# Kitsunetic/ERP_match_eightpoint_test

Hardware: AMD Instinct MI355X
Metric: ERP image-pairs/sec (4k x 4k kpts, 10k RANSAC iters); match-set bit-exact (higher is better)
Workload: dtype f32+f64; 1 GPU; configs[1] shape: 4096x4096 kpts/pair, 10000 initial_guess iters, batch of 768 independent pairs per step per GPU; kpts=4096, iters=10000, streams=6, matcher=mfma, parallelism=pair-sharded x1, sampler=glibc replay (seed 1)

## Files before the change

erp_match_eightpoint_test_amd/csrc/kernels.hip:

```cpp
#include <hip/hip_runtime.h>
#include <atomic>

#include <math.h>

#include <algorithm>
#include <type_traits>
#include <utility>
#include <stdint.h>
#include <stdlib.h>

#include "erp_device.hpp"
#include "erp_kernels.hpp"
#include "erp_launch.hpp"

namespace erp {

namespace {

constexpr float kInf = __builtin_huge_valf();

typedef float f32x2 __attribute__((ext_vector_type(2)));
typedef __attribute__((address_space(3))) uint32_t lds_u32;

__constant__ uint32_t c_red[30][31];
// ... 641 lines not shown

template <bool I24, int RS = 8>
__device__ __forceinline__ void split_hits_block(uint32_t (&ring)[31], uint32_t* bm, int lane,
                                                 int i0, int s, const uint64_t (&c)[31]) {
    const uint32_t bm_lane = (uint32_t)(size_t)(lds_u32*)bm + 4u * (uint32_t)lane;
    uint32_t jj[31];
    lat_positions<I24, true>(ring, i0, c, jj);
#pragma unroll
    for (int u = 0; u < 31; u++) {
        const uint32_t j = min(jj[u], (uint32_t)s);
        asm volatile("ds_or_b32 %0, %1" : : "v"(lds_word_addr<RS>(bm_lane, j)), "v"(1u << (j & 31))
                     : "memory");
    }
}

__device__ __forceinline__ void ring_skip_block(uint32_t (&ring)[31]) {
#pragma unroll
    for (int u = 0; u < 31; u++) {
        const int slot = 30 - u;
        ring[slot] = ring[slot] - ring[(slot + 28) % 31];
    }
}

template <typename F>
__device__ __forceinline__ void lat_blocks(int M, int s, int b0, int b1,
                                           const double* __restrict__ rtab, F&& fn) {
    uint64_t ca[31] = {}, cb[31] = {};
    auto live = [&](int b) { return b < b1 && M - 1 - 31 * b >= 1; };
    auto kind = [&](int b) { return live(b) ? lat_kind(M - 1 - 31 * b, s) : 4; };
    int b = b0;
    int ka = kind(b);
    if (live(b) && ka < 4) lat_fetch(rtab, M - 1 - 31 * b, ka, ca);
    while (live(b)) {
        const int kb = kind(b + 1);
        lat_ready(ca);
        if (live(b + 1) && kb < 4) lat_fetch(rtab, M - 1 - 31 * (b + 1), kb, cb);
        fn(b, ka, ca);
        b++;
        if (!live(b)) break;
        ka = kind(b + 1);
        lat_ready(cb);
        if (live(b + 1) && ka < 4) lat_fetch(rtab, M - 1 - 31 * (b + 1), ka, ca);
        fn(b, kb, cb);
        b++;
    }
}

__global__ __launch_bounds__(64 * (kSplitG + 1)) void sampler_split_kernel(
    const int32_t* __restrict__ counts, const uint32_t* __restrict__ wins, int nwaves, int nbw,
    double sample_frac, const double* __restrict__ rtab, uint32_t* __restrict__ selw,
    int32_t* __restrict__ flags, int nalloc) {
    extern __shared__ uint32_t sm[];
    __shared__ int esum[64];
    const int p = blockIdx.y, w = blockIdx.x, lane = threadIdx.x & 63, wv = threadIdx.x >> 6;
    const int M = counts[p];
    const int s = (int)(M * sample_frac);
    if (s < 1 || M < 2) return;
    asm volatile("s_setreg_imm32_b32 hwreg(HW_REG_MODE, 2, 2), 3\n\ts_nop 3" ::: "memory");
#if ERP_SPLIT_STAMPS
    uint64_t ts[8];
    ts[0] = __builtin_amdgcn_s_memtime();
#endif
    const size_t reg = (size_t)nalloc * 64;
    uint32_t* H = sm + (size_t)wv * reg;
    uint32_t* Bm = sm + (size_t)(kSplitG + wv) * reg;
    auto avail = [&](int k) -> uint32_t {
        return k < (s >> 5) ? ~0u : k == (s >> 5) ? (1u << (s & 31)) - 1u : 0u;
    };
    if (wv < kSplitG)
        for (int k = 0; k < nalloc; k++) H[k * 64 + lane] = 0u;
    if (wv == 0) esum[lane] = 0;
    const int nbd = M - 31 - s >= 0 ? (M - 31 - s) / 31 + 1 : 0;
    const int bb = wv < kSplitG ? nbd * wv / kSplitG : nbd;
    const int be = wv < kSplitG ? nbd * (wv + 1) / kSplitG : 0x7fffffff;
    uint32_t ring[31];
    {
        const uint32_t* wi = wins + ((size_t)p * nwaves + w) * 31 * 64 + lane;
#pragma unroll
        for (int t = 0; t < 31; t++) ring[t] = wi[t * 64];
    }
    for (int b = 0; b < bb; b++) ring_skip_block(ring);
#if ERP_SPLIT_STAMPS
    ts[1] = __builtin_amdgcn_s_memtime();
#endif
    __syncthreads();
    uint32_t ring0[31];
#pragma unroll
    for (int t = 0; t < 31; t++) ring0[t] = ring[t];
    if (wv < kSplitG)
        lat_blocks(M, s, bb, be, rtab, [&](int b, int kind, const uint64_t(&c)[31]) {
            const int i0 = M - 1 - 31 * b;
            if (kind == 0) split_hits_block<true>(ring, H, lane, i0, s, c);
            else split_hits_block<false>(ring, H, lane, i0, s, c);
        });
    asm volatile("s_waitcnt lgkmcnt(0)" ::: "memory");
#if ERP_SPLIT_STAMPS
    ts[2] = __builtin_amdgcn_s_memtime();
#endif
    __syncthreads();
#if ERP_SPLIT_STAMPS
    ts[3] = __builtin_amdgcn_s_memtime();
#endif
    const int lim = wv < kSplitG ? wv : kSplitG;
    for (int k0 = 0; k0 < nalloc; k0 += 8) {
        uint32_t e[8] = {0u, 0u, 0u, 0u, 0u, 0u, 0u, 0u};
#pragma unroll
        for (int x = 0; x < kSplitG; x++) {
            if (x < lim) {
#pragma unroll
                for (int q = 0; q < 8; q++)
                    if (k0 + q < nalloc) e[q] |= sm[(size_t)x * reg + (k0 + q) * 64 + lane];
            }
        }
#pragma unroll
        for (int q = 0; q < 8; q++)
            if (k0 + q < nalloc) Bm[(k0 + q) * 64 + lane] = avail(k0 + q) & ~e[q];
    }
#if ERP_SPLIT_STAMPS
    ts[4] = __builtin_amdgcn_s_memtime();
#endif
#pragma unroll
    for (int t = 0; t < 31; t++) ring[t] = ring0[t];
    uint32_t* out = selw + ((size_t)p * nwaves + w) * (size_t)nbw * 64 + lane;
    const int b0 = (M - 1) / 31, u0 = (M - 1) % 31;
    int emitted = 0;
    uint32_t lastw = 0;
    lat_blocks(M, s, bb, be, rtab, [&](int b, int kind, const uint64_t(&c)[31]) {
        const uint32_t word = replay_block_lat<true, 8>(ring, Bm, lane, M - 1 - 31 * b, s, kind, rtab, c);
        emitted += __builtin_popcount(word);
        if (b == b0) lastw = word;
        else out[(size_t)b * 64] = word;
    });
#if ERP_SPLIT_STAMPS
    ts[5] = __builtin_amdgcn_s_memtime();
#endif
    if (wv == kSplitG) {
        if (Bm[lane] & 1u) {
            lastw |= 1u << u0;
            emitted++;
        }
        out[(size_t)b0 * 64] = lastw;
    }
    atomicAdd(&esum[lane], emitted);
    __syncthreads();
    if (wv == kSplitG && esum[lane] != s) atomicOr(&flags[p], 2);
#if ERP_SPLIT_STAMPS
    if (blockIdx.x == 0 && blockIdx.y == 0 && lane == 0)
        printf("split wave %d: skip %d pass1 %d barrier %d init %d pass2 %d (blocks %d..%d, M %d s %d)\n",
               wv, (int)(ts[1] - ts[0]), (int)(ts[2] - ts[1]), (int)(ts[3] - ts[2]),
               (int)(ts[4] - ts[3]), (int)(ts[5] - ts[4]), bb, be, M, s);
#endif
}

__device__ __forceinline__ void philox4x32_10(uint32_t c[4], uint32_t k0, uint32_t k1) {
#pragma unroll
    for (int r = 0; r < 10; r++) {
        const uint64_t p0 = (uint64_t)0xD2511F53u * c[0], p1 = (uint64_t)0xCD9E8D57u * c[2];
        const uint32_t hi0 = (uint32_t)(p0 >> 32), lo0 = (uint32_t)p0;
        const uint32_t hi1 = (uint32_t)(p1 >> 32), lo1 = (uint32_t)p1;
        uint32_t n0, n2;
        asm("v_bitop3_b32 %0, %1, %2, %3 bitop3:0x96" : "=v"(n0) : "v"(hi1), "v"(c[1]), "s"(k0));
        asm("v_bitop3_b32 %0, %1, %2, %3 bitop3:0x96" : "=v"(n2) : "v"(hi0), "v"(c[3]), "s"(k1));
        c[0] = n0;
        c[1] = lo1;
        c[2] = n2;
        c[3] = lo0;
        k0 += 0x9E3779B9u;
        k1 += 0xBB67AE85u;
    }
}

__global__ __launch_bounds__(64) void philox_sampler_kernel(
    const int32_t* __restrict__ counts, int iters, int nwaves, int nbw, double sample_frac,
    uint32_t seed, uint64_t offset, int nwords, uint32_t* __restrict__ selw,
    int32_t* __restrict__ flags) {
    extern __shared__ uint32_t bm[];
    const int p = blockIdx.y, w = blockIdx.x, lane = wave_lane();
    const int M = counts[p];
    const int s = (int)(M * sample_frac);
    if (s < 1 || M < 2) return;
    uint32_t* out = selw + ((size_t)p * nwaves + w) * (size_t)nbw * 64 + lane;
    const int nb = (M - 1) / 31 + 1;
    if ((M + 31) / 32 > nwords) {
        if (lane == 0) atomicOr(&flags[p], 8);
        for (int b = 0; b < nb; b++) out[(size_t)b * 64] = 0u;
        return;
    }
    const int mw = (M + 31) / 32;
    for (int k = 0; k < mw; k++) bm[k * 64 + lane] = 0u;
    const uint64_t h = offset + (uint64_t)(w * 64 + lane);
    uint32_t u[4];
    for (int k0 = 0; k0 < s; k0 += 4) {
        u[0] = (uint32_t)h;
        u[1] = (uint32_t)(h >> 32);
        u[2] = (uint32_t)(k0 >> 2);
        u[3] = 0u;
        philox4x32_10(u, seed, 0x243F6A88u);
#pragma unroll
        for (int q = 0; q < 4; q++) {
            const int k = k0 + q;
            if (k < s) {
                const uint32_t j = (uint32_t)(M - s + k);
                const uint32_t t = __umulhi(u[q], j + 1u);
                const uint32_t old = atomicOr(&bm[(t >> 5) * 64 + lane], 1u << (t & 31));
                if (old & (1u << (t & 31))) atomicOr(&bm[(j >> 5) * 64 + lane], 1u << (j & 31));
            }
        }
    }
    int emitted = 0;
    for (int b = 0; b < nb; b++) {
        const int hi = M - 1 - 31 * b, lo = hi - 30;
        const int l0 = lo < 0 ? 0 : lo;
        const uint32_t a = bm[(l0 >> 5) * 64 + lane];
        const uint32_t c = ((l0 >> 5) + 1) < mw ? bm[((l0 >> 5) + 1) * 64 + lane] : 0u;
        uint32_t win = __builtin_amdgcn_alignbit(c, a, (uint32_t)(l0 & 31));
        if (lo < 0) win = (win << (-lo));
        win &= 0x7fffffffu;
        const uint32_t word = __builtin_bitreverse32(win) >> 1;
        emitted += __builtin_popcount(word);
        out[(size_t)b * 64] = word;
    }
    if (emitted != s) atomicOr(&flags[p], 2);
}

__device__ __forceinline__ void estimate_store(const double* e, double valid_abs,
                                               erp_hypothesis* __restrict__ o,
                                               bool with_e = true) {
    Hyp hy;
    estimate_from_e(e, valid_abs, hy);
#pragma unroll
    for (int k = 0; k < 3; k++) {
        o->R1[k] = hy.R1[k];
        o->R2[k] = hy.R2[k];
        o->T[k] = hy.T[k];
    }
    o->R1_valid = hy.R1_valid;
    o->R2_valid = hy.R2_valid;
    o->inliers = 0;
    if (!with_e) return;
#pragma unroll
    for (int k = 0; k < 9; k++) o->E[k] = hy.E[k];
}

constexpr int kGramLimbs = 6;
constexpr int kGramTiles = 7;
constexpr int kGramN = kGramTiles * 32;
constexpr double kGramScale = 0x1p44;

typedef int i32x4 __attribute__((ext_vector_type(4)));
typedef int i32x16 __attribute__((ext_vector_type(16)));

__device__ __forceinline__ double gram_join(int a0, int a1, int a2, int a3, int a4, int a5) {
    const double lo = __builtin_fma((double)a2, 0x1p-28,
                                    __builtin_fma((double)a1, 0x1p-36, (double)a0 * 0x1p-44));
    const double hi = __builtin_fma((double)a5, 0x1p16, __builtin_fma((double)a4, 0x1p8, (double)a3));
    return __builtin_fma(hi, 0x1p-20, lo);
}

__device__ __forceinline__ int gram_col(int limb, int c) {
    return c < 32 ? limb * 32 + c : 192 + limb * 4 + (c - 32);
}

__device__ __forceinline__ int gram_swz(int n, int u) {
    return n * 32 + ((((u >> 4) ^ (n >> 3)) & 1) << 4) + (u & 15);
}

__global__ __launch_bounds__(256) void gram_limbs_kernel(const int32_t* __restrict__ counts,
                                                         const double* __restrict__ pts,
                                                         int max_nq, int nbw,
                                                         int8_t* __restrict__ limbs) {
    __shared__ __align__(16) int8_t tile[kGramN * 32];
    const int p = blockIdx.y, b = blockIdx.x, tid = threadIdx.x;
    const int M = counts[p];
    if (M < 2 || b > (M - 1) / 31) return;
    for (int k = tid; k < kGramN * 32 / 16; k += 256)
        reinterpret_cast<uint4*>(tile)[k] = make_uint4(0u, 0u, 0u, 0u);
    __syncthreads();
    const double* P = pts + (size_t)p * (max_nq + 1) * 6;
    for (int item = tid; item < 31 * 36; item += 256) {
        const int u = item / 36, c = item - 36 * (item / 36);
        const int i = M - 1 - 31 * b - u;
        if (i < 0) continue;
        const double* pr = P + (size_t)i * 6;
        const int a = c / 6, e = c - 6 * (c / 6);
        const int ai = a < 3 ? 0 : (a < 5 ? 1 : 2), aj = a < 3 ? a : (a < 5 ? a - 2 : 2);
        const int ei = e < 3 ? 0 : (e < 5 ? 1 : 2), ej = e < 3 ? e : (e < 5 ? e - 2 : 2);
        const double LL = pr[ai] * pr[aj], RR = pr[3 + ei] * pr[3 + ej];
        long long q = __double2ll_rn((LL * RR) * kGramScale);
#pragma unroll
        for (int k = 0; k < kGramLimbs; k++) {
            const int d = (int)(int8_t)(q & 0xff);
            tile[gram_swz(gram_col(k, c), u)] = (int8_t)d;
            q = (q - d) >> 8;
        }
    }
    __syncthreads();
    uint4* o = reinterpret_cast<uint4*>(limbs + ((size_t)p * nbw + b) * kGramN * 32);
    for (int k = tid; k < kGramN * 32 / 16; k += 256) o[k] = reinterpret_cast<const uint4*>(tile)[k];
}

#ifndef ERP_GRAM_WAVES
#define ERP_GRAM_WAVES 4
#endif
#ifndef ERP_GRAM_SCHED
#define ERP_GRAM_SCHED 0
#endif
constexpr int kGramWaves = ERP_GRAM_WAVES;
constexpr int kGramWords = 2;
constexpr int kGramWordBytes = kGramN * 32;
constexpr int kGramSelOff = kGramWords * kGramWordBytes;
#ifndef ERP_GRAM_RING
#define ERP_GRAM_RING 3
#endif
#ifndef ERP_GRAM_MINBLOCKS
#define ERP_GRAM_MINBLOCKS 3
#endif
constexpr int kGramPieces = kGramSelOff / 1024;
static_assert(kGramPieces == 14, "14 limb pieces of 1 KB per step");
template <int WT>
struct GramCfg {
    static constexpr int kIters = 32 * kGramWaves * WT;
    static constexpr int kChunks = kIters / 64;
    static constexpr int kSelPW = kGramWords * kChunks / kGramWaves;
    static constexpr int kRing = WT == 1 ? ERP_GRAM_RING : 5;
    static constexpr int kSlotBytes = kGramSelOff + kGramWords * kIters * 4;
    static constexpr int kMinBlocks = WT == 1 ? ERP_GRAM_MINBLOCKS : 2;
    static_assert(kRing >= 3, "ring");
    static_assert(kIters % 64 == 0 && kGramWords * kChunks % kGramWaves == 0 && kGramWaves <= 14,
                  "whole selection-word DMAs per wave");
};
constexpr int gram_pieces_of(int w) {
    return kGramPieces / kGramWaves + (w < kGramPieces % kGramWaves ? 1 : 0);
}
constexpr int gram_piece0(int w) {
    return w * (kGramPieces / kGramWaves) + (w < kGramPieces % kGramWaves ? w : kGramPieces % kGramWaves);
}

typedef __attribute__((address_space(3))) void* lds_vptr;
typedef const __attribute__((address_space(1))) void* glb_vptr;

template <int WT>
__global__ __launch_bounds__(64 * kGramWaves, GramCfg<WT>::kMinBlocks) void gram_mfma_kernel(
    const int32_t* __restrict__ counts, const int8_t* __restrict__ limbs,
    const uint32_t* __restrict__ selw, int iters, int nwaves, int nbw, double sample_frac,
    double* __restrict__ gram, int nhb, double* __restrict__ evec,
    erp_hypothesis* __restrict__ hyps, double valid_abs) {
    using C = GramCfg<WT>;
    __shared__ __align__(16) int8_t lds[C::kRing * C::kSlotBytes];
    const int NB = gridDim.x;
    const int lbk = (NB & 7) ? (int)blockIdx.x : (int)((blockIdx.x & 7) * (NB >> 3) + (blockIdx.x >> 3));
    const int p = lbk / nhb, tid = threadIdx.x, lane = tid & 63, wv = tid >> 6;
    const int M = counts[p];
    const int s = (int)(M * sample_frac);
    if (s < 1 || M < 2) return;
    const int hb = (lbk % nhb) * C::kIters;
    if (hb >= iters) return;
    const int nb = (M - 1) / 31 + 1;
    const int nsteps = (nb + kGramWords - 1) / kGramWords;
    const int h0 = hb + wv * 32 * WT;
    const int r = lane & 31, hh = lane >> 5;
    const int8_t* lg = limbs + (size_t)p * nbw * kGramWordBytes + lane * 16;
    const int lp0 = [&] {
        int v = 0;
#pragma unroll
        for (int w = 0; w < kGramWaves; w++) v = (w == wv) ? gram_piece0(w) : v;
        return v;
    }();
    const bool extra = wv < kGramPieces % kGramWaves;
    const uint32_t* sg[C::kSelPW];
#pragma unroll
    for (int e = 0; e < C::kSelPW; e++) {
        const int d = wv * C::kSelPW + e;
        const int chunk = min((hb >> 6) + d % C::kChunks, nwaves - 1);
        sg[e] = selw + ((size_t)p * nwaves + chunk) * (size_t)nbw * 64 + lane +
                (size_t)(d / C::kChunks) * 64;
    }
    const int soff = kGramSelOff + wv * C::kSelPW * 256;
    auto issue = [&](int step) {
        const int sx = min(step, nsteps - 1);
        int8_t* slot = lds + (step % C::kRing) * C::kSlotBytes;
        const int8_t* src = lg + (size_t)sx * kGramSelOff;
#pragma unroll
        for (int k = 0; k < kGramPieces / kGramWaves; k++)
            __builtin_amdgcn_global_load_lds((glb_vptr)(src + (lp0 + k) * 1024),
                                             (lds_vptr)(slot + (lp0 + k) * 1024), 16, 0, 0);
        if (extra)
            __builtin_amdgcn_global_load_lds(
                (glb_vptr)(src + (lp0 + kGramPieces / kGramWaves) * 1024),
                (lds_vptr)(slot + (lp0 + kGramPieces / kGramWaves) * 1024), 16, 0, 0);
#pragma unroll
        for (int e = 0; e < C::kSelPW; e++)
            __builtin_amdgcn_global_load_lds((glb_vptr)(sg[e] + (size_t)(sx * kGramWords) * 64),
                                             (lds_vptr)(slot + soff + e * 256), 4, 0, 0);
    };
    i32x16 acc[WT][kGramTiles];
#pragma unroll
    for (int w = 0; w < WT; w++)
#pragma unroll
        for (int t = 0; t < kGramTiles; t++)
#pragma unroll
            for (int k = 0; k < 16; k++) acc[w][t][k] = 0;
#pragma unroll
    for (int k = 0; k < C::kRing - 1; k++) issue(k);
    const int boff = r * 32 + (((hh ^ (r >> 3)) & 1) << 4);
    for (int st = 0; st < nsteps; st++) {
        constexpr int kBase = kGramPieces / kGramWaves + C::kSelPW;
        static_assert((kBase + 1) * (C::kRing - 2) <= 63, "vmcnt range");
        if (extra) asm volatile("s_waitcnt vmcnt(%0)" ::"n"((kBase + 1) * (C::kRing - 2)) : "memory");
        else asm volatile("s_waitcnt vmcnt(%0)" ::"n"(kBase * (C::kRing - 2)) : "memory");
        __builtin_amdgcn_s_barrier();
        issue(st + C::kRing - 1);
        const int8_t* slot = lds + (st % C::kRing) * C::kSlotBytes;
        i32x4 bf[kGramWords][kGramTiles];
#pragma unroll
        for (int i = 0; i < kGramWords; i++)
#pragma unroll
            for (int t = 0; t < kGramTiles; t++)
                bf[i][t] = *reinterpret_cast<const i32x4*>(slot + i * kGramWordBytes +
                                                           t * 32 * 32 + boff);
        uint32_t wsel[WT][kGramWords];
#pragma unroll
        for (int w = 0; w < WT; w++)
#pragma unroll
            for (int i = 0; i < kGramWords; i++)
                wsel[w][i] = reinterpret_cast<const uint32_t*>(slot + kGramSelOff)[
                    i * C::kIters + (wv * WT + w) * 32 + r];
        i32x4 a[WT][kGramWords];
#pragma unroll
        for (int w = 0; w < WT; w++)
#pragma unroll
            for (int i = 0; i < kGramWords; i++) {
                const uint32_t wm = (st * kGramWords + i < nb) ? 0xffffu : 0u;
                const uint32_t bits = (wsel[w][i] >> (16 * hh)) & wm;
#pragma unroll
                for (int v = 0; v < 4; v++)
                    a[w][i][v] = (int)((((bits >> (4 * v)) & 0xfu) * 0x00204081u) & 0x01010101u);
            }
#if ERP_GRAM_SCHED
        __builtin_amdgcn_sched_group_barrier(0x100, kGramWords * (kGramTiles + 1), 0);
        __builtin_amdgcn_sched_group_barrier(0x002, 4 * kGramWords * 4, 0);
        __builtin_amdgcn_sched_group_barrier(0x008, kGramWords * kGramTiles, 0);
#endif
#pragma unroll
        for (int i = 0; i < kGramWords; i++)
#pragma unroll
            for (int t = 0; t < kGramTiles; t++)
#pragma unroll
                for (int w = 0; w < WT; w++)
                    acc[w][t] = __builtin_amdgcn_mfma_i32_32x32x32_i8(a[w][i], bf[i][t], acc[w][t], 0, 0, 0);
    }
    asm volatile("s_waitcnt vmcnt(0)" ::: "memory");
    double* go = gram + (size_t)p * 36 * iters;
    if (evec && s >= 9) {
        constexpr int kStg = C::kIters + 1;
        static_assert(36 * kStg * 8 <= C::kRing * C::kSlotBytes, "Gram stage fits the ring");
        double* stg = reinterpret_cast<double*>(lds);
        __syncthreads();
#pragma unroll
        for (int w = 0; w < WT; w++)
#pragma unroll
        for (int k = 0; k < 16; k++) {
            const int row = (wv * WT + w) * 32 + (k & 3) + 8 * (k >> 2) + 4 * hh;
            static_assert(kGramLimbs == 6, "gram_join takes six limbs");
            const int x = acc[w][kGramLimbs][k];
            int y[kGramLimbs];
#pragma unroll
            for (int t = 0; t < kGramLimbs; t++) y[t] = __shfl(x, (lane & 32) + 4 * t + (r & 3), 64);
            stg[r * kStg + row] = gram_join(acc[w][0][k], acc[w][1][k], acc[w][2][k], acc[w][3][k],
                                            acc[w][4][k], acc[w][5][k]);
            if (r < 4) stg[(32 + r) * kStg + row] = gram_join(y[0], y[1], y[2], y[3], y[4], y[5]);
        }
        __syncthreads();
        if (wv >= C::kIters / 64) return;
        const int hl = wv * 64 + lane, h = hb + hl;
        double e[9];
        const bool ok = gram_min_eigvec9_inv(stg, kStg, hl, e);
        if (h >= iters) return;
        if (!ok) {
            e[0] = __builtin_nan("");
#pragma unroll 4
            for (int k = 0; k < 36; k++) go[(size_t)k * iters + h] = stg[k * kStg + hl];
        } else if (hyps) {
            estimate_store(e, valid_abs, hyps + (size_t)p * iters + h);
            evec[(size_t)p * 9 * iters + h] = 0.0;
            return;
        }
        double* eo = evec + (size_t)p * 9 * iters + h;
#pragma unroll
        for (int k = 0; k < 9; k++) eo[(size_t)k * iters] = e[k];
        return;
    }
#pragma unroll
    for (int w = 0; w < WT; w++)
#pragma unroll
    for (int k = 0; k < 16; k++) {
        const int row = w * 32 + (k & 3) + 8 * (k >> 2) + 4 * hh;
        const int x = acc[w][kGramLimbs][k];
        int y[kGramLimbs];
#pragma unroll
        for (int t = 0; t < kGramLimbs; t++) y[t] = __shfl(x, (lane & 32) + 4 * t + (r & 3), 64);
        if (h0 + row < iters) {
            go[(size_t)r * iters + h0 + row] = gram_join(acc[w][0][k], acc[w][1][k], acc[w][2][k],
                                                         acc[w][3][k], acc[w][4][k], acc[w][5][k]);
            if (r < 4)
                go[(size_t)(32 + r) * iters + h0 + row] = gram_join(y[0], y[1], y[2], y[3], y[4], y[5]);
        }
    }
}

__global__ __launch_bounds__(64) void samples_kernel(const int32_t* __restrict__ counts,
                                                     const uint32_t* __restrict__ selw, int iters,
                                                     int nwaves, int nbw, int idx_stride,
                                                     double sample_frac,
                                                     int32_t* __restrict__ samples) {
    const int p = blockIdx.y, lane = wave_lane();
    const int h = blockIdx.x * 64 + lane;
    const int M = counts[p];
    const int s = (int)(M * sample_frac);
    if (s < 1 || M < 2 || h >= iters) return;
    const uint32_t* sp = selw + ((size_t)p * nwaves + blockIdx.x) * (size_t)nbw * 64 + lane;
    int32_t* o = samples + ((size_t)p * iters + h) * idx_stride;
    int n = 0;
    for (int b = 0; b <= (M - 1) / 31; b++) {
        uint32_t w = sp[(size_t)b * 64];
        while (w) {
            const int u = __builtin_ctz(w);
            w &= w - 1u;
            if (n < idx_stride) o[n] = M - 1 - 31 * b - u;
            n++;
        }
    }
}

__global__ __launch_bounds__(256) void gram_all_kernel(const double* __restrict__ pts, int m,
                                                       double* __restrict__ gram) {
    __shared__ double red[36][256];
    const int tid = threadIdx.x;
    double g[36];
#pragma unroll
    for (int k = 0; k < 36; k++) g[k] = 0.0;
    for (int v = tid; v < m; v += 256) {
        const double* pt = pts + (size_t)v * 6;
        const double l0 = pt[0], l1 = pt[1], l2 = pt[2], r0 = pt[3], r1 = pt[4], r2 = pt[5];
        const double LL[6] = {l0 * l0, l0 * l1, l0 * l2, l1 * l1, l1 * l2, l2 * l2};
        const double RR[6] = {r0 * r0, r0 * r1, r0 * r2, r1 * r1, r1 * r2, r2 * r2};
#pragma unroll
        for (int a = 0; a < 6; a++)
#pragma unroll
            for (int b = 0; b < 6; b++) g[6 * a + b] = __builtin_fma(LL[a], RR[b], g[6 * a + b]);
    }
#pragma unroll
    for (int k = 0; k < 36; k++) red[k][tid] = g[k];
    __syncthreads();
    for (int o = 128; o > 0; o >>= 1) {
        if (tid < o)
#pragma unroll
            for (int k = 0; k < 36; k++) red[k][tid] += red[k][tid + o];
        __syncthreads();
    }
    if (tid < 36) gram[tid] = red[tid][0];
}

template <bool THIN>
__global__ __launch_bounds__(64) void eigen_kernel(const int32_t* __restrict__ counts,
                                                   const double* __restrict__ gram, int iters,
                                                   double sample_frac,
                                                   double* __restrict__ evec,
                                                   erp_hypothesis* __restrict__ hyps,
                                                   double valid_abs) {
    const int p = blockIdx.y;
    const int h = blockIdx.x * 64 + threadIdx.x;
    const int M = counts[p];
    const int s = (int)(M * sample_frac);
    if (s < 1 || h >= iters || (s < 9) != THIN) return;
    const double* gi = gram + (size_t)p * 36 * iters + h;
    double e[9];
    if (THIN) {
        double g36[36], G[81];
#pragma unroll
        for (int k = 0; k < 36; k++) g36[k] = gi[(size_t)k * iters];
        gram36_to_full(g36, G);
        gram_jacobi9(G, s, e);
    } else if (!gram_min_eigvec9_inv(gi, iters, 0, e)) {
        e[0] = __builtin_nan("");
    }
    if (THIN && hyps) {
        estimate_store(e, valid_abs, hyps + (size_t)p * iters + h);
        return;
    }
    double* eo = evec + (size_t)p * 9 * iters + h;
#pragma unroll
    for (int k = 0; k < 9; k++) eo[(size_t)k * iters] = e[k];
}

__global__ __launch_bounds__(64) void eigen_fallback_kernel(const int32_t* __restrict__ counts,
                                                            const double* __restrict__ gram,
                                                            int iters, double sample_frac,
                                                            double* __restrict__ evec,
                                                            erp_hypothesis* __restrict__ hyps,
                                                            double valid_abs) {
    const int p = blockIdx.y;
    const int h = blockIdx.x * 64 + threadIdx.x;
    const int M = counts[p];
    const int s = (int)(M * sample_frac);
    if (s < 9 || h >= iters) return;
    double* eo = evec + (size_t)p * 9 * iters + h;
    if (!__builtin_isnan(eo[0])) return;
    double e[9];
    gram_min_eigvec9_jacobi(gram + (size_t)p * 36 * iters + h, iters, 0, e);
    if (hyps) {
        estimate_store(e, valid_abs, hyps + (size_t)p * iters + h);
        return;
    }
#pragma unroll
    for (int k = 0; k < 9; k++) eo[(size_t)k * iters] = e[k];
}

__global__ __launch_bounds__(64) void eigen_rest_kernel(const int32_t* __restrict__ counts,
                                                        const double* __restrict__ gram, int iters,
                                                        double sample_frac,
                                                        double* __restrict__ evec,
                                                        erp_hypothesis* __restrict__ hyps,
                                                        double valid_abs) {
    const int p = blockIdx.y;
    const int h = blockIdx.x * 64 + threadIdx.x;
    const int M = counts[p];
    const int s = (int)(M * sample_frac);
    if (s < 1 || h >= iters) return;
    double* eo = evec + (size_t)p * 9 * iters + h;
    const double* gi = gram + (size_t)p * 36 * iters + h;
    double e[9];
    if (s < 9) {
        double g36[36], G[81];
#pragma unroll
        for (int k = 0; k < 36; k++) g36[k] = gi[(size_t)k * iters];
        gram36_to_full(g36, G);
        gram_jacobi9(G, s, e);
    } else {
        if (!__builtin_isnan(eo[0])) return;
        gram_min_eigvec9_jacobi(gi, iters, 0, e);
    }
    if (hyps) {
        estimate_store(e, valid_abs, hyps + (size_t)p * iters + h);
        return;
    }
#pragma unroll
    for (int k = 0; k < 9; k++) eo[(size_t)k * iters] = e[k];
}

#ifdef ERP_EST_WAVES
#define ERP_EST_ATTR __attribute__((amdgpu_waves_per_eu(ERP_EST_WAVES)))
#else
#define ERP_EST_ATTR
#endif
__global__ __launch_bounds__(64) ERP_EST_ATTR void estimate_kernel(const int32_t* __restrict__ counts,
                                                      const double* __restrict__ evec, int iters,
                                                      double sample_frac, double valid_abs,
                                                      erp_hypothesis* __restrict__ hyps,
                                                      int with_e) {
    const int p = blockIdx.y;
    const int h = blockIdx.x * 64 + threadIdx.x;
    const int M = counts[p];
    const int s = (int)(M * sample_frac);
    if (s < 1 || h >= iters) return;
    const double* ei = evec + (size_t)p * 9 * iters + h;
    double e[9];
#pragma unroll
    for (int k = 0; k < 9; k++) e[k] = ei[(size_t)k * iters];
    estimate_store(e, valid_abs, hyps + (size_t)p * iters + h, with_e != 0);
}

template <bool REST>
__global__ __launch_bounds__(64) ERP_EST_ATTR void estimate_lite_kernel(
    const int32_t* __restrict__ counts, const double* __restrict__ evec, int iters,
    double sample_frac, double valid_abs, float* __restrict__ hl, int32_t* __restrict__ wsum,
    const double* __restrict__ gram) {
    const int p = blockIdx.y, w = blockIdx.x, lane = threadIdx.x;
    const int h = w * 64 + lane;
    const int M = counts[p];
    const int s = (int)(M * sample_frac);
    if (s < 1) return;
    Hyp hy;
    hy.R1_valid = hy.R2_valid = 0;
    if (h < iters) {
        const double* ei = evec + (size_t)p * 9 * iters + h;
        double e[9];
#pragma unroll
        for (int k = 0; k < 9; k++) e[k] = ei[(size_t)k * iters];
        if (REST) {
            const double* gi = gram + (size_t)p * 36 * iters + h;
            if (s < 9) {
                double g36[36], G[81];
#pragma unroll
                for (int k = 0; k < 36; k++) g36[k] = gi[(size_t)k * iters];
                gram36_to_full(g36, G);
                gram_jacobi9(G, s, e);
            } else if (__builtin_isnan(e[0])) {
                gram_min_eigvec9_jacobi(gi, iters, 0, e);
            }
        }
        estimate_from_e(e, valid_abs, hy);
        float* o = hl + (size_t)p * 9 * iters + h;
        const float qnan = __builtin_nanf("");
        o[0] = hy.R1_valid ? hy.R1[0] : qnan;
        o[(size_t)1 * iters] = hy.R1[1];
        o[(size_t)2 * iters] = hy.R1[2];
        o[(size_t)3 * iters] = hy.R2_valid ? hy.R2[0] : qnan;
        o[(size_t)4 * iters] = hy.R2[1];
        o[(size_t)5 * iters] = hy.R2[2];
#pragma unroll
        for (int k = 0; k < 3; k++) o[(size_t)(6 + k) * iters] = hy.T[k];
    }
    int cnt = (hy.R1_valid != 0) + (hy.R2_valid != 0);
    float mn[3] = {kInf, kInf, kInf}, mx[3] = {-kInf, -kInf, -kInf};
#pragma unroll
    for (int k = 0; k < 3; k++) {
        if (hy.R1_valid) {
            mn[k] = fminf(mn[k], hy.R1[k]);
            mx[k] = fmaxf(mx[k], hy.R1[k]);
        }
        if (hy.R2_valid) {
            mn[k] = fminf(mn[k], hy.R2[k]);
            mx[k] = fmaxf(mx[k], hy.R2[k]);
        }
    }
#pragma unroll
    for (int o = 32; o > 0; o >>= 1) {
        cnt += __shfl_xor(cnt, o, 64);
#pragma unroll
        for (int k = 0; k < 3; k++) {
            mn[k] = fminf(mn[k], __shfl_xor(mn[k], o, 64));
            mx[k] = fmaxf(mx[k], __shfl_xor(mx[k], o, 64));
        }
    }
    if (lane < 8) {
        const int32_t v = lane == 0 ? cnt : lane < 4 ? __float_as_int(mn[lane - 1])
                          : lane < 7 ? __float_as_int(mx[lane - 4]) : 0;
        wsum[((size_t)p * gridDim.x + w) * 8 + lane] = v;
    }
}

__device__ __forceinline__ int hyp_valid_count(const erp_hypothesis& hy) {
    return (hy.R1_valid != 0) + (hy.R2_valid != 0);
}

__global__ __launch_bounds__(1024) void valid_count_kernel(const int32_t* __restrict__ counts,
                                                           const erp_hypothesis* __restrict__ hyps,
                                                           int iters, double sample_frac,
                                                           int32_t* __restrict__ vchunk) {
    __shared__ int ws[16];
    __shared__ float red6[6][16];
    const int p = blockIdx.y, c = blockIdx.x, tid = threadIdx.x;
    const int M = counts[p];
    if ((int)(M * sample_frac) < 1) return;
// ... 3118 lines not shown
```

Measured before the change: 42470 pairs/s.

## Software-pipeline Gram MFMA loop with rolling LDS fragment reads and buffer DMAs

Restructures the Gram MFMA inner step so that B fragments are read from LDS through a rolling window of kQuads registers, with explicit lgkmcnt waits placed between MFMAs instead of loading all fragments up front. The next step's global-to-LDS DMAs are interleaved one per MFMA, and they now use buffer resources (raw_ptr_buffer_load_lds) in place of flat global pointers. Selection words are read as 16-bit halves and uniform values are hoisted with readfirstlane. The aim is to overlap LDS reads and DMA issue with MFMA execution and to lower register pressure, at the cost of hand-written asm waits that must track the exact instruction counts.

```diff
diff --git a/erp_match_eightpoint_test_amd/csrc/kernels.hip b/erp_match_eightpoint_test_amd/csrc/kernels.hip
--- a/erp_match_eightpoint_test_amd/csrc/kernels.hip
+++ b/erp_match_eightpoint_test_amd/csrc/kernels.hip
@@ -967,9 +967,6 @@
 #ifndef ERP_GRAM_WAVES
 #define ERP_GRAM_WAVES 4
 #endif
-#ifndef ERP_GRAM_SCHED
-#define ERP_GRAM_SCHED 0
-#endif
 constexpr int kGramWaves = ERP_GRAM_WAVES;
 constexpr int kGramWords = 2;
 constexpr int kGramWordBytes = kGramN * 32;
@@ -979,6 +976,12 @@
 #endif
 #ifndef ERP_GRAM_MINBLOCKS
 #define ERP_GRAM_MINBLOCKS 3
+#endif
+#ifndef ERP_GRAM_QUADS1
+#define ERP_GRAM_QUADS1 4
+#endif
+#ifndef ERP_GRAM_QUADS2
+#define ERP_GRAM_QUADS2 2
 #endif
 constexpr int kGramPieces = kGramSelOff / 1024;
 static_assert(kGramPieces == 14, "14 limb pieces of 1 KB per step");
@@ -990,6 +993,8 @@
     static constexpr int kRing = WT == 1 ? ERP_GRAM_RING : 5;
     static constexpr int kSlotBytes = kGramSelOff + kGramWords * kIters * 4;
     static constexpr int kMinBlocks = WT == 1 ? ERP_GRAM_MINBLOCKS : 2;
+    static constexpr int kQuads = WT == 1 ? ERP_GRAM_QUADS1 : ERP_GRAM_QUADS2;
+    static_assert(kQuads >= 2 && kQuads <= kGramPieces, "at least one read ahead");
     static_assert(kRing >= 3, "ring");
     static_assert(kIters % 64 == 0 && kGramWords * kChunks % kGramWaves == 0 && kGramWaves <= 14,
                   "whole selection-word DMAs per wave");
@@ -1002,7 +1007,84 @@
 }
 
 typedef __attribute__((address_space(3))) void* lds_vptr;
-typedef const __attribute__((address_space(1))) void* glb_vptr;
+constexpr int kBufRsrcFlags = 0x00020000;
+
+template <int WT>
+struct GramDma {
+    using C = GramCfg<WT>;
+    static constexpr int kP = kGramPieces / kGramWaves;
+    static constexpr int kOps = kP + 1 + C::kSelPW;
+    __amdgpu_buffer_rsrc_t lrs, srs[C::kSelPW];
+    int8_t* lds;
+    int lane16, lane4, lp0, soff, nsteps;
+    bool extra;
+    template <int J>
+    __device__ __forceinline__ void op(int step) const {
+        const int sx = min(step, nsteps - 1);
+        int8_t* slot = lds + (step % C::kRing) * C::kSlotBytes;
+        if constexpr (J <= kP) {
+            if (J < kP || extra)
+                __builtin_amdgcn_raw_ptr_buffer_load_lds(lrs, (lds_vptr)(slot + (lp0 + J) * 1024), 16,
+                                                         lane16, sx * kGramSelOff + (lp0 + J) * 1024,
+                                                         0, 0);
+        } else {
+            constexpr int e = J - kP - 1;
+            __builtin_amdgcn_raw_ptr_buffer_load_lds(srs[e], (lds_vptr)(slot + soff + e * 256), 4,
+                                                     lane4, sx * kGramWords * 256, 0, 0);
+        }
+    }
+    template <int J = 0>
+    __device__ __forceinline__ void all(int step) const {
+        if constexpr (J < kOps) {
+            op<J>(step);
+            all<J + 1>(step);
+        }
+    }
+};
+
+template <int F>
+__device__ __forceinline__ void gram_frag_read(i32x4& q, uint32_t addr) {
+    asm volatile("ds_read_b128 %0, %1 offset:%2" : "=v"(q) : "v"(addr), "n"(F * 1024) : "memory");
+}
+template <int N>
+__device__ __forceinline__ void gram_frag_wait(i32x4& q) {
+    asm volatile("s_waitcnt lgkmcnt(%1)" : "+v"(q) : "n"(N));
+}
+template <int NQ, int F = 0>
+__device__ __forceinline__ void gram_step_reads(i32x4 (&q)[NQ], uint32_t addr) {
+    if constexpr (F < NQ) {
+        gram_frag_read<F>(q[F], addr);
+        gram_step_reads<NQ, F + 1>(q, addr);
+    }
+}
+template <int WT, int NQ, int F>
+__device__ __forceinline__ void gram_step_frag(i32x16 (&acc)[WT][kGramTiles],
+                                               uint32_t (&wsel)[WT][kGramWords],
+                                               const uint32_t (&wm)[kGramWords], i32x4 (&a)[WT],
+                                               i32x4 (&q)[NQ], uint32_t addr,
+                                               const GramDma<WT>& dma, int dstep) {
+    if constexpr (F < kGramPieces) {
+        if constexpr (F % kGramTiles == 0) {
+#pragma unroll
+            for (int w = 0; w < WT; w++) {
+                asm volatile("" : "+v"(wsel[w][F / kGramTiles]));
+                const uint32_t bits = wsel[w][F / kGramTiles] & wm[F / kGramTiles];
+#pragma unroll
+                for (int v = 0; v < 4; v++)
+                    a[w][v] = (int)((((bits >> (4 * v)) & 0xfu) * 0x00204081u) & 0x01010101u);
+            }
+        }
+        constexpr int kLeft = kGramPieces - 1 - F;
+        gram_frag_wait<(kLeft < NQ - 1 ? kLeft : NQ - 1)>(q[F % NQ]);
+#pragma unroll
+        for (int w = 0; w < WT; w++)
+            acc[w][F % kGramTiles] = __builtin_amdgcn_mfma_i32_32x32x32_i8(
+                a[w], q[F % NQ], acc[w][F % kGramTiles], 0, 0, 0);
+        if constexpr (F + NQ < kGramPieces) gram_frag_read<F + NQ>(q[F % NQ], addr);
+        if constexpr (F < GramDma<WT>::kOps) dma.template op<F>(dstep);
+        gram_step_frag<WT, NQ, F + 1>(acc, wsel, wm, a, q, addr, dma, dstep);
+    }
+}
 
 template <int WT>
 __global__ __launch_bounds__(64 * kGramWaves, GramCfg<WT>::kMinBlocks) void gram_mfma_kernel(
@@ -1014,50 +1096,40 @@
     __shared__ __align__(16) int8_t lds[C::kRing * C::kSlotBytes];
     const int NB = gridDim.x;
     const int lbk = (NB & 7) ? (int)blockIdx.x : (int)((blockIdx.x & 7) * (NB >> 3) + (blockIdx.x >> 3));
-    const int p = lbk / nhb, tid = threadIdx.x, lane = tid & 63, wv = tid >> 6;
+    const int p = lbk / nhb, tid = threadIdx.x, kl = tid & 63;
+    const int wv = __builtin_amdgcn_readfirstlane(tid >> 6);
     const int M = counts[p];
-    const int s = (int)(M * sample_frac);
+    const int s = __builtin_amdgcn_readfirstlane((int)(M * sample_frac));
     if (s < 1 || M < 2) return;
     const int hb = (lbk % nhb) * C::kIters;
     if (hb >= iters) return;
     const int nb = (M - 1) / 31 + 1;
     const int nsteps = (nb + kGramWords - 1) / kGramWords;
     const int h0 = hb + wv * 32 * WT;
-    const int r = lane & 31, hh = lane >> 5;
-    const int8_t* lg = limbs + (size_t)p * nbw * kGramWordBytes + lane * 16;
-    const int lp0 = [&] {
-        int v = 0;
-#pragma unroll
-        for (int w = 0; w < kGramWaves; w++) v = (w == wv) ? gram_piece0(w) : v;
-        return v;
-    }();
-    const bool extra = wv < kGramPieces % kGramWaves;
-    const uint32_t* sg[C::kSelPW];
+    const int kr = kl & 31, kh = kl >> 5;
+    GramDma<WT> dma;
+    dma.lds = lds;
+    dma.nsteps = nsteps;
+    dma.lane16 = kl * 16;
+    dma.lane4 = kl * 4;
+    dma.lrs = __builtin_amdgcn_make_buffer_rsrc(
+        const_cast<int8_t*>(limbs + (size_t)p * nbw * kGramWordBytes), 0, nbw * kGramWordBytes,
+        kBufRsrcFlags);
+    dma.lp0 = 0;
+#pragma unroll
+    for (int w = 0; w < kGramWaves; w++) dma.lp0 = (w == wv) ? gram_piece0(w) : dma.lp0;
+    dma.extra = wv < kGramPieces % kGramWaves;
 #pragma unroll
     for (int e = 0; e < C::kSelPW; e++) {
         const int d = wv * C::kSelPW + e;
         const int chunk = min((hb >> 6) + d % C::kChunks, nwaves - 1);
-        sg[e] = selw + ((size_t)p * nwaves + chunk) * (size_t)nbw * 64 + lane +
-                (size_t)(d / C::kChunks) * 64;
-    }
-    const int soff = kGramSelOff + wv * C::kSelPW * 256;
-    auto issue = [&](int step) {
-        const int sx = min(step, nsteps - 1);
-        int8_t* slot = lds + (step % C::kRing) * C::kSlotBytes;
-        const int8_t* src = lg + (size_t)sx * kGramSelOff;
-#pragma unroll
-        for (int k = 0; k < kGramPieces / kGramWaves; k++)
-            __builtin_amdgcn_global_load_lds((glb_vptr)(src + (lp0 + k) * 1024),
-                                             (lds_vptr)(slot + (lp0 + k) * 1024), 16, 0, 0);
-        if (extra)
-            __builtin_amdgcn_global_load_lds(
-                (glb_vptr)(src + (lp0 + kGramPieces / kGramWaves) * 1024),
-                (lds_vptr)(slot + (lp0 + kGramPieces / kGramWaves) * 1024), 16, 0, 0);
-#pragma unroll
-        for (int e = 0; e < C::kSelPW; e++)
-            __builtin_amdgcn_global_load_lds((glb_vptr)(sg[e] + (size_t)(sx * kGramWords) * 64),
-                                             (lds_vptr)(slot + soff + e * 256), 4, 0, 0);
-    };
+        dma.srs[e] = __builtin_amdgcn_make_buffer_rsrc(
+            const_cast<uint32_t*>(selw + ((size_t)p * nwaves + chunk) * (size_t)nbw * 64 +
+                                  (size_t)(d / C::kChunks) * 64),
+            0, (nbw - d / C::kChunks) * 256, kBufRsrcFlags);
+    }
+    dma.soff = kGramSelOff + wv * C::kSelPW * 256;
+    const bool extra = dma.extra;
     i32x16 acc[WT][kGramTiles];
 #pragma unroll
     for (int w = 0; w < WT; w++)
@@ -1066,55 +1138,35 @@
 #pragma unroll
             for (int k = 0; k < 16; k++) acc[w][t][k] = 0;
 #pragma unroll
-    for (int k = 0; k < C::kRing - 1; k++) issue(k);
-    const int boff = r * 32 + (((hh ^ (r >> 3)) & 1) << 4);
+    for (int k = 0; k < C::kRing - 1; k++) dma.all(k);
+    const int boff = kr * 32 + (((kh ^ (kr >> 3)) & 1) << 4);
+    const int woff = kr * 4 + kh * 2;
     for (int st = 0; st < nsteps; st++) {
         constexpr int kBase = kGramPieces / kGramWaves + C::kSelPW;
         static_assert((kBase + 1) * (C::kRing - 2) <= 63, "vmcnt range");
         if (extra) asm volatile("s_waitcnt vmcnt(%0)" ::"n"((kBase + 1) * (C::kRing - 2)) : "memory");
         else asm volatile("s_waitcnt vmcnt(%0)" ::"n"(kBase * (C::kRing - 2)) : "memory");
         __builtin_amdgcn_s_barrier();
-        issue(st + C::kRing - 1);
         const int8_t* slot = lds + (st % C::kRing) * C::kSlotBytes;
-        i32x4 bf[kGramWords][kGramTiles];
-#pragma unroll
-        for (int i = 0; i < kGramWords; i++)
-#pragma unroll
-            for (int t = 0; t < kGramTiles; t++)
-                bf[i][t] = *reinterpret_cast<const i32x4*>(slot + i * kGramWordBytes +
-                                                           t * 32 * 32 + boff);
         uint32_t wsel[WT][kGramWords];
 #pragma unroll
         for (int w = 0; w < WT; w++)
 #pragma unroll
             for (int i = 0; i < kGramWords; i++)
-                wsel[w][i] = reinterpret_cast<const uint32_t*>(slot + kGramSelOff)[
-                    i * C::kIters + (wv * WT + w) * 32 + r];
-        i32x4 a[WT][kGramWords];
-#pragma unroll
-        for (int w = 0; w < WT; w++)
-#pragma unroll
-            for (int i = 0; i < kGramWords; i++) {
-                const uint32_t wm = (st * kGramWords + i < nb) ? 0xffffu : 0u;
-                const uint32_t bits = (wsel[w][i] >> (16 * hh)) & wm;
-#pragma unroll
-                for (int v = 0; v < 4; v++)
-                    a[w][i][v] = (int)((((bits >> (4 * v)) & 0xfu) * 0x00204081u) & 0x01010101u);
-            }
-#if ERP_GRAM_SCHED
-        __builtin_amdgcn_sched_group_barrier(0x100, kGramWords * (kGramTiles + 1), 0);
-        __builtin_amdgcn_sched_group_barrier(0x002, 4 * kGramWords * 4, 0);
-        __builtin_amdgcn_sched_group_barrier(0x008, kGramWords * kGramTiles, 0);
-#endif
-#pragma unroll
-        for (int i = 0; i < kGramWords; i++)
-#pragma unroll
-            for (int t = 0; t < kGramTiles; t++)
-#pragma unroll
-                for (int w = 0; w < WT; w++)
-                    acc[w][t] = __builtin_amdgcn_mfma_i32_32x32x32_i8(a[w][i], bf[i][t], acc[w][t], 0, 0, 0);
+                wsel[w][i] = *reinterpret_cast<const uint16_t*>(
+                    slot + kGramSelOff + (i * C::kIters + (wv * WT + w) * 32) * 4 + woff);
+        const uint32_t wm[kGramWords] = {0xffffu,
+                                         (st * kGramWords + 1 < nb) ? 0xffffu : 0u};
+        static_assert(kGramWords == 2, "wm");
+        const uint32_t baddr = (uint32_t)(uintptr_t)(lds_vptr)(slot + boff);
+        i32x4 bq[C::kQuads];
+        gram_step_reads<C::kQuads>(bq, baddr);
+        i32x4 a[WT];
+        gram_step_frag<WT, C::kQuads, 0>(acc, wsel, wm, a, bq, baddr, dma, st + C::kRing - 1);
     }
     asm volatile("s_waitcnt vmcnt(0)" ::: "memory");
+    const int lane = __builtin_amdgcn_mbcnt_hi(~0u, __builtin_amdgcn_mbcnt_lo(~0u, 0u));
+    const int r = lane & 31, hh = lane >> 5;
     double* go = gram + (size_t)p * 36 * iters;
     if (evec && s >= 9) {
         constexpr int kStg = C::kIters + 1;
```

Measured after the change: 43920 pairs/s (median of 6 runs). 3.4% higher.
